# garrelt/C2-Ray3Dm1D_Helium

Measured on AMD Instinct MI355X. Metric: cell-updates/sec (grid_cells x sources x iters / wall) on 256^3 box; % HBM roofline, higher is better.
Workload: dtype f64

## Files before the change

### __graft_entry__.py

```python
from __future__ import annotations

import importlib.util
import subprocess
import sys
from pathlib import Path

ROOT = Path(__file__).resolve().parent
PKG_DIR = ROOT / "c2-ray3dm1d_helium_amd"
PKG_NAME = "c2ray_helium_amd"
PARAMS_VARIANT = {"subboxsize": 4, "max_subbox": 9, "convergence_fraction": "1.0e-3"}


def load_package():
    if PKG_NAME in sys.modules:
        return sys.modules[PKG_NAME]
    spec = importlib.util.spec_from_file_location(PKG_NAME, PKG_DIR / "__init__.py",
                                                  submodule_search_locations=[str(PKG_DIR)])
    mod = importlib.util.module_from_spec(spec)
    sys.modules[PKG_NAME] = mod
    spec.loader.exec_module(mod)
    return mod


def build() -> None:
    pkg = load_package()
    lib = pkg.build(force=False)
    assert lib.exists(), lib
    subprocess.run(["make", "-C", str(ROOT / "oracle"), "liboracle.so", "liboracle_params.so"], check=True)
    alt = PKG_DIR / "libc2ray_hip_params.so"
    deps = pkg._build.SOURCES + pkg._build.HEADERS
    if not alt.exists() or alt.stat().st_mtime < max(p.stat().st_mtime for p in deps):
        pkg._build.build(params=PARAMS_VARIANT, out=alt)
    subprocess.run(["g++", "-O2", "-ffp-contract=off", "-mfma", "-fPIC", "-shared", "-std=c++17", "-o",
                    str(ROOT / "tests" / "_host_harness.so"), str(ROOT / "tests" / "host_harness.cpp")], check=True)
    from c2ray_helium_amd import _build
    for name, flags in (("gpu_func_probe", ["-O3"]), ("fake_rccl", ["-O2", "-pthread"]), ("fake_rccl_corrupt", ["-O2", "-pthread"])):
        src, so = ROOT / "tests" / f"{name}.hip", ROOT / "tests" / f"_{name}.so"
        deps = [src] + (list((PKG_DIR / "csrc").glob("*.hpp")) if name == "gpu_func_probe" else [])
        if name == "fake_rccl_corrupt":
            deps.append(ROOT / "tests" / "fake_rccl.hip")
        if not so.exists() or so.stat().st_mtime < max(p.stat().st_mtime for p in deps):
            subprocess.run([_build.hipcc(), "--offload-arch=gfx950", *flags, "-ffp-contract=off", "-fPIC", "-shared", "-std=c++17", "-o",
                            str(so), str(src)], check=True)
    for variant in (["16"], ["16", "pl"], ["16", "lls"], ["16", "cubep3m"], ["16", "params"], ["64", "omp"], ["256", "omp", "timer"]):
        subprocess.run([str(ROOT / "oracle" / "ref_build.sh"), *variant], check=True)
    import ctypes
    so = ctypes.CDLL(str(lib))
    for name in pkg._lib.SYMBOLS:
        getattr(so, name)


def smoke() -> None:
    import numpy as np
    pkg = load_package()
    sys.path.insert(0, str(ROOT / "oracle"))
    import oracle as orc

    z = np.load(ROOT / "tests" / "golden" / "tap_N16_heat_3src.npz")
    g = lambda k: z["c1_in_" + k]
    tables = pkg.RadiationTables.load()
    mesh = tuple(int(m) for m in g("mesh"))
    mat = pkg.Material(ndens=g("ndens"), xh=g("xh").copy(), xhe=g("xhe").copy(),
                       temperature_grid=g("temperature").copy(), isothermal=False,
                       temper_val=float(g("temper_val")[0]), clumping=float(g("clumping")[0]), reccoef=g("reccoef"))
    grid = pkg.GridProps(mesh, tuple(g("dr")), float(g("vol")[0]))
    src = pkg.SourceProps(g("srcpos").reshape(-1, 3), g("NormFlux"), float(g("S_star")[0]))
    cosmo = pkg.Cosmology(float(g("zred")[0]), float(g("H0")[0]), float(g("Omega0")[0]))
    ev = pkg.Evolve(mesh, tables, device=0)
    e = ev.engine
    e.set_step(mat, grid, cosmo)
    e.set_sources(src)
    e.upload_state(mat)
    e.begin_step()
    e.set_rates_to_zero()
    e.pass_sources(1, 1)
    conv = e.global_pass(float(g("dt")[0]))
    got = {**e.download_rates(), **e.download_iter_state()}

    with np.load(pkg.evolve.DEFAULT_TABLES) as t:
        T = orc.Tables({k: t[k] for k in t.files})
    st = orc.Step(mesh, g("dr"), g("vol")[0], g("zred")[0], g("H0")[0], g("Omega0")[0], 0, g("temper_val")[0],
                  g("clumping")[0], g("srcpos"), g("NormFlux"), g("S_star")[0], g("ndens"), g("reccoef"))
    s = orc.State(st, g("xh"), g("xhe"), g("temperature"))
    orc.begin_step(s)
    orc.pass_all_sources(T, st, s)
    conv_ref = orc.global_pass(T, st, s, float(g("dt")[0]))
    worst = 0.0
    for k, ref in [("phih_grid", s.phih), ("phihe_grid", s.phihe), ("phiheat", s.phiheat), ("xh_av", s.xh_av),
                   ("xhe_av", s.xhe_av), ("xh_intermed", s.xh_intermed)]:
        rel = np.abs(got[k] - ref) / np.maximum(np.abs(ref), 1e-300)
        worst = max(worst, float(rel.max()))
    print(f"smoke: 16^3 x 3 sources, heating: conv_flag gpu={conv} oracle={conv_ref}, worst rel diff {worst:.3e}")
    assert conv == conv_ref, (conv, conv_ref)
    assert worst == 0.0, worst


if __name__ == "__main__":
    build()
    print("build ok")
```

### c2-ray3dm1d_helium_amd/csrc/c2ray_hip.hip

```cpp
#include <hip/hip_runtime.h>

#include <algorithm>
#include <atomic>
#include <chrono>
#include <cmath>
#include <cstdarg>
#include <cstdio>
#include <cstdlib>
#include <cstring>
#include <string>
#include <thread>
#include <type_traits>
#include <unordered_map>
#include <vector>

#include "../../include/c2ray_hip.h"
#include "c2ray_device.hpp"
#include "c2ray_shell.hpp"

using namespace c2r;

namespace {

constexpr int BATCH_MAX = 4096;
// ... 341 lines not shown
  const StepScalars &sc = A.sc;
  int di, dj, dk;
  ReachShell RS{};
  if constexpr (OPEN) RS = reach_shell(S.rl, S.rr, G.s);
  const int face = OPEN ? reach_decode(RS, t, di, dj, dk) : shell_decode_fast(G, t, di, dj, dk);
  Box cut_;
  if constexpr (OPEN) cut_ = source_box(A.box, S);
  const Box &box = OPEN ? cut_ : A.box;
  const bool inside = di >= box.lo[0] && di <= box.hi[0] && dj >= box.lo[1] && dj <= box.hi[1] && dk >= box.lo[2] &&
                      dk <= box.hi[2];
  if (!inside) return;
  const size_t cz = S.cz;
  const size_t p = (OPEN ? (size_t)RS.off : (size_t)G.off) + (size_t)t;
  global_double *cs = (global_double *)S.cols;
  const int i = mesh0<OPEN>(S.i0 - 1 + di, g.n1), j = mesh0<OPEN>(S.j0 - 1 + dj, g.n2), k = mesh0<OPEN>(S.k0 - 1 + dk, g.n3);
  double u_HI, u_HeI, u_HeII;
  sweep_cell_state(A, i, j, k, face == 2, u_HI, u_HeI, u_HeII);
  ShellCorners c4;
  if constexpr (OPEN) reach_short_characteristic(G, reach_shell(S.rl, S.rr, G.sp), S.rl, S.rr, face, S.i0, S.j0, S.k0, di, dj, dk, c4);
  else shell_short_characteristic(G, face, S.i0, S.j0, S.k0, di, dj, dk, c4);
  double cin_HI = interp_column_fast(c4.s, cs[col_out((size_t)c4.p[0], 0, cz)], cs[col_out((size_t)c4.p[1], 0, cz)],
                                     cs[col_out((size_t)c4.p[2], 0, cz)], cs[col_out((size_t)c4.p[3], 0, cz)], sigma_HI_at_ion_freq);
  const double cin_HeI = interp_column_fast(c4.s, cs[col_out((size_t)c4.p[0], 1, cz)], cs[col_out((size_t)c4.p[1], 1, cz)],
                                            cs[col_out((size_t)c4.p[2], 1, cz)], cs[col_out((size_t)c4.p[3], 1, cz)], sigma_HeI_at_ion_freq);
  const double cin_HeII = interp_column_fast(c4.s, cs[col_out((size_t)c4.p[0], 2, cz)], cs[col_out((size_t)c4.p[1], 2, cz)],
                                             cs[col_out((size_t)c4.p[2], 2, cz)], cs[col_out((size_t)c4.p[3], 2, cz)], sigma_HeII_at_ion_freq);
  const double path = c4.path * sc.dr1;
  if (sc.use_lls) {
    const double coldensh_LLS =
        A.lls_grid ? (double)A.lls_grid[(size_t)i + (size_t)g.n1 * ((size_t)j + (size_t)g.n2 * (size_t)k)] : sc.coldensh_lls;
    cin_HI = cin_HI + coldensh_LLS * path / sc.dr1;
  }
  const double cout_HI = cin_HI + u_HI * path * (1.0 - abu_he);
  const double cout_HeI = cin_HeI + u_HeI * path * abu_he;
  const double cout_HeII = cin_HeII + u_HeII * path * abu_he;
  store_columns(cs, p, cz, cin_HI, cin_HeI, cin_HeII, cout_HI, cout_HeI, cout_HeII);
}

__device__ __forceinline__ int sweep_block_cell(int cnt) {
  const int nblk_shell = (cnt + BLOCK - 1) / BLOCK;
  int vb = (int)blockIdx.x;
  if ((gridDim.x & 7u) == 0) {
    const int chunk = (int)gridDim.x >> 3;
    vb = ((int)blockIdx.x & 7) * chunk + ((int)blockIdx.x >> 3);
  }
  if (vb >= nblk_shell) return -1;
  const int t = vb * BLOCK + (int)threadIdx.x;
  return t < cnt ? t : -1;
}

__device__ __forceinline__ int sweep_block_cell_open(int cnt) {
  const int nblk_shell = (cnt + BLOCK - 1) / BLOCK;
  int vb = (int)blockIdx.x;
  if (nblk_shell >= 64) {
    const int chunk = (nblk_shell + 7) >> 3;
    if (vb >= 8 * chunk) return -1;
    vb = (vb & 7) * chunk + (vb >> 3);
  }
  if (vb >= nblk_shell) return -1;
  const int t = vb * BLOCK + (int)threadIdx.x;
  return t < cnt ? t : -1;
}

template <bool OPEN>
__device__ __forceinline__ int sweep_shell_cells(const SrcDev &S, int shell) {
  if constexpr (OPEN) return (int)(reach_cells(S.rl, S.rr, shell) - reach_cells(S.rl, S.rr, shell - 1));
  else return (int)shell_count(shell);
}

template <bool OPEN>
__global__ void __launch_bounds__(BLOCK, C2R_SWEEP_WAVES)
k_sweep_shell(SweepArgs A, const SrcDev *__restrict__ src, const int *__restrict__ active, int shell) {
  const SrcDev &S = src[active[blockIdx.y]];
  const int t = OPEN ? sweep_block_cell_open(sweep_shell_cells<OPEN>(S, shell)) : sweep_block_cell((int)shell_count(shell));
  if (t >= 0) sweep_cell<OPEN>(A, S, shell, t);
}

template <bool OPEN>
__global__ void __launch_bounds__(BLOCK, C2R_SWEEP_WAVES)
k_sweep_shell_fast(SweepArgs A, const SrcDev *__restrict__ src, const int *__restrict__ active, ShellGeom G) {
  const SrcDev &S = src[active[blockIdx.y]];
  const int t = OPEN ? sweep_block_cell_open(sweep_shell_cells<OPEN>(S, G.s)) : sweep_block_cell(24 * G.s * G.s + 2);
  if (t >= 0) sweep_cell_fast<OPEN>(A, S, G, t);
}

__global__ void __launch_bounds__(BLOCK)
k_loss_finish(const double *__restrict__ loss_partial, int pitch, int count, double *__restrict__ loss_acc) {
  __shared__ double sh[BLOCK / 64];
  const double *p = loss_partial + (size_t)blockIdx.x * pitch;
  double a = 0.0;
  for (int i = threadIdx.x; i < count; i += BLOCK) a += p[i];
  const double tot = block_sum(a, sh);
  if (threadIdx.x == 0) loss_acc[blockIdx.x] = tot;
}

struct ProbeRound {
  int s_lo, s_hi;
  Box box;
  int list_off;
  int nact;
  int nblk;
  int partial_off;
  int acc_off;
};
template <bool OPEN>
__global__ void __launch_bounds__(BLOCK)
k_loss_probe_rounds(Grid g, const SrcDev *__restrict__ src, const int *__restrict__ lists, const ProbeRound *__restrict__ rounds,
                    int multi, StepScalars sc, const BandData *__restrict__ bd, SedSet ss, const int *__restrict__ block_base,
                    double *__restrict__ loss_partial, int sample) {
  __shared__ double sh[BLOCK / 64];
  const ProbeRound &R = rounds[blockIdx.z];
  if ((int)blockIdx.x >= R.nblk || (int)blockIdx.y >= R.nact) return;
  const SrcDev &S = src[lists[R.list_off + blockIdx.y]];
  Box cut_;
  if constexpr (OPEN) cut_ = source_box(R.box, S);
  const Box &box = OPEN ? cut_ : R.box;
  const int s_lo = R.s_lo, s_hi = R.s_hi;
  const int B = block_base[s_hi + 1] - 1 - (int)blockIdx.x * sample;
  int lo = s_lo, hi = s_hi;
  while (lo < hi) {
    const int mid = (lo + hi + 1) >> 1;
    if (block_base[mid] <= B) lo = mid; else hi = mid - 1;
  }
  const int shell = lo;
  ReachShell RS{};
  if constexpr (OPEN) RS = reach_shell(S.rl, S.rr, shell);
  const long long cnt = OPEN ? (long long)RS.cnt : shell_count(shell);
  const int slot = threadIdx.x & 31;
  const long long t = (long long)(B - block_base[shell]) * BLOCK + (threadIdx.x >> 5) * 32;
  double loss = 0.0;
  if (t < cnt) {
    int di, dj, dk;
    if constexpr (OPEN) reach_decode(RS, (int)t, di, dj, dk);
    else shell_decode(shell, (int)t, di, dj, dk);
    const bool inside = di >= box.lo[0] && di <= box.hi[0] && dj >= box.lo[1] && dj <= box.hi[1] && dk >= box.lo[2] &&
                        dk <= box.hi[2];
    const bool boundary = on_counted_face<OPEN>(box, S, di, dj, dk, 1);
    if (inside && boundary) {
      const size_t cz = S.cz;
      const size_t p = (OPEN ? (size_t)RS.off : (size_t)shell_offset(shell)) + (size_t)t;
      const global_double *cs = (const global_double *)S.cols;
      const double cin_HI = cs[col_in(p, 0, cz)], cin_HeI = cs[col_in(p, 1, cz)], cin_HeII = cs[col_in(p, 2, cz)];
      const double cout_HI = cs[col_out(p, 0, cz)], cout_HeI = cs[col_out(p, 1, cz)], cout_HeII = cs[col_out(p, 2, cz)];
      if (cin_HI < max_coldensh) {
        double vol_ph;
        if (shell == 0) {
          vol_ph = sc.dr1 * sc.dr2 * sc.dr3;
        } else {
          const double path = sc_path(di, dj, dk) * sc.dr1;
          const double xs = sc.dr1 * (double)di, ys = sc.dr2 * (double)dj, zs = sc.dr3 * (double)dk;
          vol_ph = 4.0 * pi * (xs * xs + ys * ys + zs * zs) * path;
        }
        const double nf[NSED] = {S.nflux, S.nflux_sed[0], S.nflux_sed[1]};
        double po = 0.0;
        for (int sd = 0; sd < (multi ? NSED : 1); sd++) {
          if (!(nf[sd] > 0.0)) continue;
          for (int b = ss.lo[sd] + slot; b < ss.hi[sd]; b += 32)
            po += photo_out_band(*bd, sd, ss.photo_thick[sd], ss.photo_thin[sd], b, cin_HI, cout_HI, cin_HeI, cout_HeI, cin_HeII,
                                 cout_HeII, nf[sd]);
        }
        loss = po * sc.vol / vol_ph;
      }
    }
  }
  const double bs = block_sum(loss, sh);
  if (threadIdx.x == 0) loss_partial[(size_t)R.partial_off + (size_t)blockIdx.y * R.nblk + blockIdx.x] = bs;
// ... 2112 lines not shown
  }
  HIPCHK(c, hipMemcpyAsync(c->d_src[set], hs, sizeof(SrcDev) * B.nb, hipMemcpyHostToDevice, c->stream));
  return 0;
}

static int settle_rounds(const PassCtx &P, Batch &B) {
  c2r_ctx *c = P.c;
  if (B.settled == B.recs.size()) return 0;
  if (launch_probes(P, B)) return 1;
  HIPCHK(c, hipEventSynchronize(c->ev_probe));
  int *hl = c->h_list[B.set];
  for (; B.settled < B.recs.size(); B.settled++) {
    const RoundRec &R = B.recs[B.settled];
    const double *probe = c->h_probe + R.acc_off;
    const int *lst = hl + R.off;
    std::vector<int> undecided;
    for (int a = 0; a < R.nact; a++) {
      SrcRun &r = B.run[lst[a]];
      if (!r.active) continue;
      r.loss = probe[a];
      if (!(r.loss > 2.0 * (C2R_F(1e-10) * r.total_flux))) undecided.push_back(lst[a]);
    }
    if (!undecided.empty()) {
      int *ul = hl + B.list_used;
      std::copy(undecided.begin(), undecided.end(), ul);
      HIPCHK(c, hipMemcpyAsync(c->d_list[B.set] + B.list_used, ul, sizeof(int) * undecided.size(), hipMemcpyHostToDevice, c->stream));
      if (boundary_loss(c, B.set, B.list_used, (int)undecided.size(), R.s_lo, R.s_hi, R.box, P.sc, P.ss, P.multi, true)) return 1;
      B.list_used += undecided.size();
      for (size_t j = 0; j < undecided.size(); j++) B.run[undecided[j]].loss = c->h_loss[j];
    }
    for (int a = 0; a < R.nact; a++) {
      SrcRun &r = B.run[lst[a]];
      if (!r.active) continue;
      if (!(r.loss > C2R_F(1e-10) * r.total_flux)) {
        r.active = false;
        r.nbox = R.round;
      }
    }
  }
  return 0;
}

static bool all_reached(const c2r_ctx *c, const Batch &B, int round) {
  for (const SrcRun &r : B.run)
    if (r.active && c->prev_nbox[(size_t)r.ns - 1] < round) return false;
  return true;
}

static int move_block(const PassCtx &P, Batch &B, int b, int ncap, double *ncols) {
  c2r_ctx *c = P.c;
  SrcRun &r = B.run[b];
  if (B.launched > B.settled) HIPCHK(c, hipStreamWaitEvent(c->stream, c->ev_probe, 0));
  SrcDev &S = c->h_src[B.set][b];
  const size_t ncz = source_block_entries(c, r.ns, ncap);
  const size_t have = r.smax_prev >= 0 ? source_block_entries(c, r.ns, r.smax_prev) : 0;
  for (int half = 0; half < 2 && have > 0; half++)
    HIPCHK(c, hipMemcpyAsync(ncols + 3 * half * ncz, S.cols + 3 * half * S.cz, sizeof(double) * 3 * have,
                             hipMemcpyDeviceToDevice, c->stream));
  if (S.cz > 0) c->vacated[B.set].push_back(c2r_ctx::Segment{S.cols, 6 * S.cz});
  S.cols = ncols;
  S.cz = ncz;
  r.cap = ncap;
  c->arena_stats[3]++;
  HIPCHK(c, hipMemcpyAsync(c->d_src[B.set] + b, &S, sizeof(SrcDev), hipMemcpyHostToDevice, c->stream));
  return 0;
}

static int start_over(const PassCtx &P, Batch &B, int round) {
  c2r_ctx *c = P.c;
  HIPCHK(c, hipStreamSynchronize(c->stream));
  HIPCHK(c, hipStreamSynchronize(c->stream_probe));
  const int limit_rounds = (c->g.smax + SUBBOXSIZE - 1) / SUBBOXSIZE;
  for (const SrcRun &r : B.run) {
    int &pn = c->prev_nbox[(size_t)r.ns - 1];
    pn = std::max(pn, r.active ? limit_rounds : r.nbox);
  }
  if (B.nb == 1) return fail(c, "column scratch: one source of this mesh does not fit in device memory");
  if (P.arena_log) fprintf(stderr, "c2ray_hip: column scratch, set %d: no room to grow in round %d, batch of %d starts over\n", B.set, round, B.nb);
  if (B.restarts++ > 0) B.nb = (B.nb + 1) / 2;
  c->arena_stats[4]++;
  return START_OVER;
}

static int launch_shells(PassCtx &P, Batch &B, const Box &box, int s_lo, int s_hi, size_t act_off, int nact) {
  c2r_ctx *c = P.c;
  SweepArgs SA;
  SA.g = c->g; SA.box = box; SA.sc = P.sc;
  SA.ndens = c->d_ndens; SA.xh_av = c->d_xh_av; SA.xhe_av = c->d_xhe_av;
  SA.lls_grid = c->lls_on_grid ? c->d_lls : nullptr;
  const int *act = c->h_list[B.set] + act_off;
  if (c->timing && !B.sweep_started) {
    HIPCHK(c, hipEventRecord(B.ev[0], c->stream));
    B.sweep_started = true;
  }
  for (int s = s_lo; s <= s_hi; s++) {
    if ((s >= TRANSPOSED_FROM_SHELL || B.nb > 16) && !P.transposed_seen) {
      HIPCHK(c, hipStreamWaitEvent(c->stream, c->ev_transposed, 0));
      P.transposed_seen = true;
    }
    SA.packed = SA.packedT = nullptr;
    if (P.transposed_seen || P.packed_early) SA.packed = c->d_stateT;
    if (P.transposed_seen) SA.packedT = c->d_stateT + 3 * c->g.ncell;
    int nblk = c->block_base[s + 1] - c->block_base[s];
    if (!c->periodic) {
      long long most = 0;
      for (int a = 0; a < nact; a++) {
        const Reach &R = B.run[act[a]].reach;
        most = std::max(most, reach_cells(R.l, R.r, s) - reach_cells(R.l, R.r, s - 1));
      }
      nblk = (int)((most + BLOCK - 1) / BLOCK);
      if (nblk == 0) continue;
    }
    const int nlaunch = nblk >= 64 ? ((nblk + 7) & ~7) : nblk;
    for (int a = 0; a < nact; a++)
      if (s <= B.run[act[a]].smax) B.run[act[a]].sweep_threads += (long long)nlaunch * BLOCK;
    const bool fast = s >= 2 && (s <= SHELL_FAST_MAX || !c->periodic) && !P.generic_sweep;
    if (fast && c->periodic)
      hipLaunchKernelGGL(k_sweep_shell_fast<false>, dim3(nlaunch, nact), dim3(BLOCK), 0, c->stream, SA, c->d_src[B.set],
                         c->d_list[B.set] + act_off, c->shell_geom[(size_t)s]);
    else if (fast)
      hipLaunchKernelGGL(k_sweep_shell_fast<true>, dim3(nlaunch, nact), dim3(BLOCK), 0, c->stream, SA, c->d_src[B.set],
                         c->d_list[B.set] + act_off, c->shell_geom[(size_t)s]);
    else if (c->periodic)
      hipLaunchKernelGGL(k_sweep_shell<false>, dim3(nlaunch, nact), dim3(BLOCK), 0, c->stream, SA, c->d_src[B.set], c->d_list[B.set] + act_off, s);
    else
      hipLaunchKernelGGL(k_sweep_shell<true>, dim3(nlaunch, nact), dim3(BLOCK), 0, c->stream, SA, c->d_src[B.set], c->d_list[B.set] + act_off, s);
    c->tm.sweep_launches++;
  }
  HIPCHK(c, hipGetLastError());
  return 0;
}

static int sweep_batch(PassCtx &P, Batch &B) {
  c2r_ctx *c = P.c;
  const Reach &reach = P.reach;
  B.list_used = 0;
  B.recs.clear();
  B.settled = B.launched = 0;
  B.sweep_started = false;
  const size_t acc_need = (size_t)B.nb * (size_t)(c->g.smax / SUBBOXSIZE + 3);
  if (c->probe_acc_cap < acc_need) {
    HIPCHK(c, hipStreamSynchronize(c->stream_probe));
    if (ensure_pair<double>(c, &c->d_probe_acc, &c->h_probe, &c->probe_acc_cap, acc_need)) return 1;
  }
  int *hl = c->h_list[B.set];
  size_t cur_off = 0;
  int cur_nact = 0;
  size_t acc_used = 0;
  for (int round = 1;; round++) {
    const Box box = round_box(reach, round);
    int s_hi = 0;
    const bool ahead = round > 1 && cur_nact > 0 && all_reached(c, B, round);
    if (!ahead && settle_rounds(P, B)) return 1;
    int nact = 0;
    int *act = hl + B.list_used;
    int s_lo = 1 << 30;
    for (int b = 0; b < B.nb; b++) {
      SrcRun &r = B.run[b];
      if (!r.active) continue;
      if (!can_grow(c, r.reach, round_box(r.reach, r.nbox)) || !(ahead || r.loss > C2R_F(1e-10) * r.total_flux)) {
        r.active = false;
        continue;
      }
      r.nbox = round;
      act[nact++] = b;
      s_lo = std::min(s_lo, r.smax_prev + 1);
      s_hi = std::max(s_hi, box_smax(round_box(r.reach, round)));
    }
    if (nact == 0) return settle_rounds(P, B);
    if (s_hi > c->g.smax) return fail(c, "internal: shell %d beyond smax %d", s_hi, c->g.smax);
    for (int a = 0; a < nact; a++) {
      const int cap = B.run[act[a]].cap;
      const int need = std::min(s_hi, B.run[act[a]].smax);
      if (cap >= need) continue;
      const int ncap = std::min(B.run[act[a]].smax, std::max(need, 2 * cap));
      double *ncols = arena_alloc(c, B.set, source_block_doubles(c, B.run[act[a]].ns, ncap));
      if (!ncols) return start_over(P, B, round);
      if (move_block(P, B, act[a], ncap, ncols)) return 1;
    }
    size_t act_off = B.list_used;
    if (cur_nact == nact && round > 1 && std::equal(act, act + nact, hl + cur_off)) {
      act_off = cur_off;
    } else {
      HIPCHK(c, hipMemcpyAsync(c->d_list[B.set] + B.list_used, act, sizeof(int) * nact, hipMemcpyHostToDevice, c->stream));
      B.list_used += (size_t)nact;
    }
    cur_off = act_off;
    cur_nact = nact;
    if (launch_shells(P, B, box, s_lo, s_hi, act_off, nact)) return 1;
    bool any_can_grow = false, any_can_grow_twice = false;
    for (int a = 0; a < nact; a++) {
      SrcRun &r = B.run[hl[act_off + a]];
      r.smax_prev = std::min(s_hi, r.smax);
      any_can_grow = any_can_grow || can_grow(c, r.reach, round_box(r.reach, round));
      any_can_grow_twice = any_can_grow_twice || can_grow(c, r.reach, round_box(r.reach, round + 1));
    }
    if (!any_can_grow) {
      if (settle_rounds(P, B)) return 1;
      for (int a = 0; a < nact; a++) {
        SrcRun &r = B.run[hl[act_off + a]];
        if (!r.active) continue;
        r.final_loss_due = true;
        r.active = false;
      }
      return 0;
    }
    RoundRec R;
    R.round = round; R.nact = nact; R.s_lo = s_lo; R.s_hi = s_hi; R.off = act_off; R.acc_off = acc_used; R.box = box;
    acc_used += (size_t)nact;
    B.recs.push_back(R);
// ... 1122 lines not shown
```

### c2-ray3dm1d_helium_amd/csrc/c2ray_shell.hpp

```cpp
#pragma once

#include <stdint.h>

#include "c2ray_device.hpp"

namespace c2r {

C2R_HD long long shell_count(int s) { return s == 0 ? 1 : 24LL * s * s + 2; }

C2R_HD long long shell_offset(int s) { return s == 0 ? 0 : (long long)(2 * s - 1) * (2 * s - 1) * (2 * s - 1); }

C2R_HD void shell_decode(int s, int t, int &di, int &dj, int &dk) {
  if (s == 0) { di = dj = dk = 0; return; }
  const int w = 2 * s + 1, v = 2 * s - 1;
  const int A = w * w, B = v * w, C = v * v;
  if (t < 2 * A) {
    dk = t < A ? s : -s;
    if (t >= A) t -= A;
    dj = t / w - s;
    di = t % w - s;
  } else if (t < 2 * A + 2 * B) {
    t -= 2 * A;
    dj = t < B ? s : -s;
    if (t >= B) t -= B;
// ... 69 lines not shown
  const int s = G.s;
  const int face = t < 2 * G.A ? 0 : (t < 2 * G.A + 2 * G.B ? 1 : 2);
  const int first = face == 0 ? 0 : (face == 1 ? 2 * G.A : 2 * G.A + 2 * G.B);
  const int size = face == 0 ? G.A : (face == 1 ? G.B : G.C);
  const int width = face == 2 ? G.v : G.w;
  const uint32_t magic = face == 2 ? G.mv : G.mw;
  const int shift = face == 2 ? G.kv : G.kw;
  const int tf = t - first;
  const bool neg = tf >= size;
  const uint32_t u = (uint32_t)(neg ? tf - size : tf);
  const uint32_t r = mulhi_u32(u, magic) >> shift;
  const int col = (int)(u - r * (uint32_t)width);
  const int a = col - (face == 2 ? s - 1 : s);
  const int b = (int)r - (face == 0 ? s : s - 1);
  const int c = neg ? -s : s;
  di = face == 2 ? c : a;
  dj = face == 0 ? b : (face == 1 ? c : a);
  dk = face == 0 ? c : b;
  return face;
}

C2R_HD int position_in_previous_shell(const ShellGeom &G, int i, int j, int k) {
  const int sp = G.sp;
  const int ja = j < 0 ? -j : j, ka = k < 0 ? -k : k;
  const int tk = (k > 0 ? 0 : G.Ap) + (j + sp) * G.wp + (i + sp);
  const int tj = 2 * G.Ap + (j > 0 ? 0 : G.Bp) + (k + sp - 1) * G.wp + (i + sp);
  const int ti = 2 * G.Ap + 2 * G.Bp + (i > 0 ? 0 : G.Cp) + (k + sp - 1) * G.vp + (j + sp - 1);
  return ka == sp ? tk : (ja == sp ? tj : ti);
}

struct ShellCorners {
  uint32_t p[4];
  double s[4];
  double path;
};
C2R_HD void shell_short_characteristic(const ShellGeom &G, int face, int i0, int j0, int k0, int di, int dj, int dk,
                                       ShellCorners &sc) {
  const int sp = G.sp;
  const int da = face == 2 ? dj : di, db = face == 0 ? dj : dk;
  const int a0 = face == 2 ? j0 : i0, b0 = face == 0 ? j0 : k0;
  const int sga = da >= 0 ? 1 : -1, sgb = db >= 0 ? 1 : -1;
  const int am = da - sga, bm = db - sgb;
  const double fa = (double)da, fb = (double)db;
  const double ac = G.alam * fa + (double)a0, bc = G.alam * fb + (double)b0;
  const double ea = 2.0 * fabs(ac - ((double)(a0 + am) + 0.5 * sga));
  const double eb = 2.0 * fabs(bc - ((double)(b0 + bm) + 0.5 * sgb));
  sc.s[0] = (1. - ea) * (1. - eb);
  sc.s[1] = (1. - eb) * ea;
  sc.s[2] = (1. - ea) * eb;
  sc.s[3] = ea * eb;
  const double num = fa * fa + fb * fb;
  const double q0 = num * G.rn2;
  const double quo = __builtin_fma(__builtin_fma(-G.n2, q0, num), G.rn2, q0);
  sc.path = sqrt(quo + 1.0);
  const int ca = da > sp ? sp : (da < -sp ? -sp : da), cb = db > sp ? sp : (db < -sp ? -sp : db);
  const uint32_t offp = (uint32_t)G.offp;
  if (face == 0) {
    const int km = dk > 0 ? sp : -sp;
    const int base = (km > 0 ? 0 : G.Ap) + sp;
    const int ra = base + (bm + sp) * G.wp, rb = base + (cb + sp) * G.wp;
    sc.p[0] = offp + (uint32_t)(ra + am);
    sc.p[1] = offp + (uint32_t)(ra + ca);
    sc.p[2] = offp + (uint32_t)(rb + am);
    sc.p[3] = offp + (uint32_t)(rb + ca);
  } else if (face == 1) {
    const int jm = dj > 0 ? sp : -sp;
    const int rk_base = (jm + sp) * G.wp + sp, rj_base = 2 * G.Ap + (jm > 0 ? 0 : G.Bp) + sp + (sp - 1) * G.wp;
    const int bma = bm < 0 ? -bm : bm, cba = cb < 0 ? -cb : cb;
    const int ra = bma == sp ? (bm > 0 ? 0 : G.Ap) + rk_base : rj_base + bm * G.wp;
    const int rb = cba == sp ? (cb > 0 ? 0 : G.Ap) + rk_base : rj_base + cb * G.wp;
    sc.p[0] = offp + (uint32_t)(ra + am);
    sc.p[1] = offp + (uint32_t)(ra + ca);
    sc.p[2] = offp + (uint32_t)(rb + am);
    sc.p[3] = offp + (uint32_t)(rb + ca);
  } else {
    const int im = di > 0 ? sp : -sp;
    sc.p[0] = offp + (uint32_t)position_in_previous_shell(G, im, am, bm);
    sc.p[1] = offp + (uint32_t)position_in_previous_shell(G, im, ca, bm);
    sc.p[2] = offp + (uint32_t)position_in_previous_shell(G, im, am, cb);
    sc.p[3] = offp + (uint32_t)position_in_previous_shell(G, im, ca, cb);
  }
}

C2R_HD int reach_lo(int l, int s) { return l > -s ? l : -s; }
C2R_HD int reach_hi(int r, int s) { return r < s ? r : s; }
C2R_HD long long reach_cells(const int *l, const int *r, int s) {
  if (s < 0) return 0;
  long long e = 1;
  for (int d = 0; d < 3; d++) e *= (long long)(reach_hi(r[d], s) - reach_lo(l[d], s) + 1);
  return e;
}

struct ReachShell {
  int s;
  int lox, loy;
  int loyp, lozp;
  int ex, eyp;
  int b1, b2, b3, b4, b5;
  int cnt;
  uint32_t off;
};
C2R_HD ReachShell reach_shell(const int *l, const int *r, int s) {
  ReachShell G;
  G.s = s;
  G.lox = reach_lo(l[0], s);
  G.loy = reach_lo(l[1], s);
  G.ex = reach_hi(r[0], s) - G.lox + 1;
  const int ey = reach_hi(r[1], s) - G.loy + 1;
  if (s == 0) {
    G.loyp = G.lozp = 0;
    G.eyp = 1;
    G.b1 = G.b2 = G.b3 = G.b4 = G.b5 = G.cnt = 1;
    G.off = 0;
    return G;
  }
  G.loyp = reach_lo(l[1], s - 1);
  G.lozp = reach_lo(l[2], s - 1);
  G.eyp = reach_hi(r[1], s - 1) - G.loyp + 1;
  const int exp_ = reach_hi(r[0], s - 1) - reach_lo(l[0], s - 1) + 1;
  const int ezp = reach_hi(r[2], s - 1) - G.lozp + 1;
  const int A = G.ex * ey, B = G.ex * ezp, C = G.eyp * ezp;
  G.b1 = s <= r[2] ? A : 0;
  G.b2 = G.b1 + (s <= -l[2] ? A : 0);
  G.b3 = G.b2 + (s <= r[1] ? B : 0);
  G.b4 = G.b3 + (s <= -l[1] ? B : 0);
  G.b5 = G.b4 + (s <= r[0] ? C : 0);
  G.cnt = G.b5 + (s <= -l[0] ? C : 0);
  G.off = (uint32_t)(exp_ * G.eyp * ezp);
  return G;
}

C2R_HD int reach_decode(const ReachShell &G, int t, int &di, int &dj, int &dk) {
  const int s = G.s;
  const int face = t < G.b2 ? 0 : (t < G.b4 ? 1 : 2);
  const int first = face == 0 ? 0 : (face == 1 ? G.b2 : G.b4);
  const int mid = face == 0 ? G.b1 : (face == 1 ? G.b3 : G.b5);
  const int width = face == 2 ? G.eyp : G.ex;
  const bool neg = t >= mid;
  const uint32_t u = (uint32_t)(t - (neg ? mid : first));
  const uint32_t row = u / (uint32_t)width;
  const int col = (int)(u - row * (uint32_t)width);
  const int a = col + (face == 2 ? G.loyp : G.lox);
  const int b = (int)row + (face == 0 ? G.loy : G.lozp);
  const int c = neg ? -s : s;
  di = face == 2 ? c : a;
  dj = face == 0 ? b : (face == 1 ? c : a);
  dk = face == 0 ? c : b;
  return face;
}

C2R_HD int reach_position_in_shell(const ReachShell &G, int i, int j, int k) {
  const int s = G.s;
  const int ja = j < 0 ? -j : j, ka = k < 0 ? -k : k;
  const int tk = (k > 0 ? 0 : G.b1) + (j - G.loy) * G.ex + (i - G.lox);
  const int tj = (j > 0 ? G.b2 : G.b3) + (k - G.lozp) * G.ex + (i - G.lox);
  const int ti = (i > 0 ? G.b4 : G.b5) + (k - G.lozp) * G.eyp + (j - G.loyp);
  return s == 0 ? 0 : (ka == s ? tk : (ja == s ? tj : ti));
}

C2R_HD size_t reach_position(const int *l, const int *r, int di, int dj, int dk) {
  const int ia = di < 0 ? -di : di, ja = dj < 0 ? -dj : dj, ka = dk < 0 ? -dk : dk;
  const int s = ia > ja ? (ia > ka ? ia : ka) : (ja > ka ? ja : ka);
  const ReachShell G = reach_shell(l, r, s);
  return (size_t)G.off + (size_t)reach_position_in_shell(G, di, dj, dk);
}

// ... 63 lines not shown
```

Measured before the change: 5.909 billion.

## Fuse groups of consecutive shells into one blocked sweep kernel with LDS hand-off

Adds a kernel that processes K (2 or 4) consecutive shells per launch for periodic fast sweeps. Each block owns a tile of the outermost shell, recomputes its upstream halo on inner shells, and passes column densities between shells through shared memory instead of reloading them from global memory. This cuts the number of kernel launches and the global traffic for the upstream columns. The cost is redundant halo recomputation and extra shared-memory use, which may lower occupancy.

```diff
diff --git a/__graft_entry__.py b/__graft_entry__.py
--- a/__graft_entry__.py
+++ b/__graft_entry__.py
@@ -31,8 +31,9 @@
     deps = pkg._build.SOURCES + pkg._build.HEADERS
     if not alt.exists() or alt.stat().st_mtime < max(p.stat().st_mtime for p in deps):
         pkg._build.build(params=PARAMS_VARIANT, out=alt)
-    subprocess.run(["g++", "-O2", "-ffp-contract=off", "-mfma", "-fPIC", "-shared", "-std=c++17", "-o",
-                    str(ROOT / "tests" / "_host_harness.so"), str(ROOT / "tests" / "host_harness.cpp")], check=True)
+    for name in ("host_harness", "sweep_blocked_harness"):
+        subprocess.run(["g++", "-O2", "-ffp-contract=off", "-mfma", "-fPIC", "-shared", "-std=c++17", "-o",
+                        str(ROOT / "tests" / f"_{name}.so"), str(ROOT / "tests" / f"{name}.cpp")], check=True)
     from c2ray_helium_amd import _build
     for name, flags in (("gpu_func_probe", ["-O3"]), ("fake_rccl", ["-O2", "-pthread"]), ("fake_rccl_corrupt", ["-O2", "-pthread"])):
         src, so = ROOT / "tests" / f"{name}.hip", ROOT / "tests" / f"_{name}.so"
diff --git a/c2-ray3dm1d_helium_amd/csrc/c2ray_hip.hip b/c2-ray3dm1d_helium_amd/csrc/c2ray_hip.hip
--- a/c2-ray3dm1d_helium_amd/csrc/c2ray_hip.hip
+++ b/c2-ray3dm1d_helium_amd/csrc/c2ray_hip.hip
@@ -447,6 +447,111 @@
   const SrcDev &S = src[active[blockIdx.y]];
   const int t = OPEN ? sweep_block_cell_open(sweep_shell_cells<OPEN>(S, G.s)) : sweep_block_cell(24 * G.s * G.s + 2);
   if (t >= 0) sweep_cell_fast<OPEN>(A, S, G, t);
+}
+
+template <int K>
+struct ShellGroup { ShellGeom G[K]; };
+
+__device__ __forceinline__ int sweep_block_tile(int ntiles) {
+  int vb = (int)blockIdx.x;
+  if ((gridDim.x & 7u) == 0) {
+    const int chunk = (int)gridDim.x >> 3;
+    vb = ((int)blockIdx.x & 7) * chunk + ((int)blockIdx.x >> 3);
+  }
+  return vb < ntiles ? vb : -1;
+}
+
+template <bool FIRST>
+__device__ __forceinline__ void sweep_cell_blocked(const SweepArgs &A, const SrcDev &S, const ShellGeom &G, int f, int a, int b, int c,
+                                                   bool owned, const double *in, int in_pitch, const PatchRect &P, double &o_HI,
+                                                   double &o_HeI, double &o_HeII) {
+  const Grid &g = A.g;
+  const StepScalars &sc = A.sc;
+  const Box &box = A.box;
+  int di, dj, dk;
+  plane_cell(f, a, b, c, di, dj, dk);
+  o_HI = o_HeI = o_HeII = 0.0;
+  const bool inside = di >= box.lo[0] && di <= box.hi[0] && dj >= box.lo[1] && dj <= box.hi[1] && dk >= box.lo[2] &&
+                      dk <= box.hi[2];
+  if (!inside) return;
+  const int face = shell_face(G, dj, dk);
+  const size_t cz = S.cz;
+  global_double *cs = (global_double *)S.cols;
+  const int i = wrap0(S.i0 - 1 + di, g.n1), j = wrap0(S.j0 - 1 + dj, g.n2), k = wrap0(S.k0 - 1 + dk, g.n3);
+  double u_HI, u_HeI, u_HeII;
+  sweep_cell_state(A, i, j, k, f == 2, u_HI, u_HeI, u_HeII);
+  ShellCorners c4;
+  shell_short_characteristic(G, face, S.i0, S.j0, S.k0, di, dj, dk, c4);
+  double n[3][4];
+  if constexpr (FIRST) {
+#pragma unroll
+    for (int x = 0; x < 3; x++)
+#pragma unroll
+      for (int q = 0; q < 4; q++) n[x][q] = cs[col_out((size_t)c4.p[q], x, cz)];
+  } else {
+    int slot[4];
+    shell_corner_slots(G, face, f, P, di, dj, dk, slot);
+#pragma unroll
+    for (int x = 0; x < 3; x++)
+#pragma unroll
+      for (int q = 0; q < 4; q++) n[x][q] = in[x * in_pitch + slot[q]];
+  }
+  double cin_HI = interp_column_fast(c4.s, n[0][0], n[0][1], n[0][2], n[0][3], sigma_HI_at_ion_freq);
+  const double cin_HeI = interp_column_fast(c4.s, n[1][0], n[1][1], n[1][2], n[1][3], sigma_HeI_at_ion_freq);
+  const double cin_HeII = interp_column_fast(c4.s, n[2][0], n[2][1], n[2][2], n[2][3], sigma_HeII_at_ion_freq);
+  const double path = c4.path * sc.dr1;
+  if (sc.use_lls) {
+    const double coldensh_LLS =
+        A.lls_grid ? (double)A.lls_grid[(size_t)i + (size_t)g.n1 * ((size_t)j + (size_t)g.n2 * (size_t)k)] : sc.coldensh_lls;
+    cin_HI = cin_HI + coldensh_LLS * path / sc.dr1;
+  }
+  o_HI = cin_HI + u_HI * path * (1.0 - abu_he);
+  o_HeI = cin_HeI + u_HeI * path * abu_he;
+  o_HeII = cin_HeII + u_HeII * path * abu_he;
+  if (owned && face == f)
+    store_columns(cs, (size_t)G.off + (size_t)position_in_shell(G, di, dj, dk), cz, cin_HI, cin_HeI, cin_HeII, o_HI, o_HeI, o_HeII);
+}
+
+template <int K>
+__global__ void __launch_bounds__(BLOCK, 6)
+k_sweep_shells_blocked(SweepArgs A, const SrcDev *__restrict__ src, const int *__restrict__ active, ShellGroup<K> GG) {
+  constexpr int TA = SWEEP_TILE_A, TB = sweep_tile_b(K);
+  constexpr int N0 = sweep_patch_cells(K, K - 1), N1 = K > 2 ? sweep_patch_cells(K, K - 2) : 1;
+  static_assert(N0 <= 2 * BLOCK && 3 * (N0 + N1) * sizeof(double) <= 16384, "two handed-over shells in 16 KB");
+  __shared__ double hand0[3 * N0], hand1[3 * N1];
+  const SrcDev &S = src[active[blockIdx.y]];
+  const int s_last = GG.G[K - 1].s;
+  const int tile = sweep_block_tile(sweep_tile_count(s_last, TA, TB));
+  if (tile < 0) return;
+  int f, sgn;
+  PatchRect T;
+  sweep_tile(s_last, TA, TB, tile, f, sgn, T);
+#pragma unroll 1
+  for (int m = 0; m < K; m++) {
+    const ShellGeom &G = GG.G[m];
+    PatchRect Q = T;
+    for (int s = s_last; s > G.s; s--) Q = upstream_rect(Q, s - 1);
+    const PatchRect P = upstream_rect(Q, G.sp);
+    const int na = Q.ahi - Q.alo + 1, cells = na * (Q.bhi - Q.blo + 1);
+    const uint32_t magic = patch_magic(na);
+    double *out = (m & 1) ? hand1 : hand0;
+    const double *in = (m & 1) ? hand0 : hand1;
+    const int out_pitch = (m & 1) ? N1 : N0, in_pitch = (m & 1) ? N0 : N1;
+    for (int idx = (int)threadIdx.x; idx < cells; idx += BLOCK) {
+      const int row = patch_row(idx, magic);
+      const int a = Q.alo + (idx - row * na), b = Q.blo + row;
+      const bool owned = a >= T.alo && a <= T.ahi && b >= T.blo && b <= T.bhi;
+      double o_HI, o_HeI, o_HeII;
+      if (m == 0) sweep_cell_blocked<true>(A, S, G, f, a, b, sgn * G.s, owned, in, in_pitch, P, o_HI, o_HeI, o_HeII);
+      else sweep_cell_blocked<false>(A, S, G, f, a, b, sgn * G.s, owned, in, in_pitch, P, o_HI, o_HeI, o_HeII);
+      if (m < K - 1) {
+        out[idx] = o_HI;
+        out[out_pitch + idx] = o_HeI;
+        out[2 * out_pitch + idx] = o_HeII;
+      }
+    }
+    if (m < K - 1) __syncthreads();
+  }
 }
 
 __global__ void __launch_bounds__(BLOCK)
@@ -2725,6 +2830,20 @@
   return START_OVER;
 }
 
+struct SweepBlocking { int from, K; };
+static const SweepBlocking SWEEP_BLOCKING[] = {{2, 4}, {64, 1}};
+static int sweep_blocking_row(int s) {
+  int r = 0;
+  for (int i = 0; i < (int)(sizeof SWEEP_BLOCKING / sizeof SWEEP_BLOCKING[0]); i++)
+    if (s >= SWEEP_BLOCKING[i].from) r = i;
+  return r;
+}
+static int sweep_blocking(int s) { return s < SWEEP_BLOCKING[0].from ? 1 : SWEEP_BLOCKING[sweep_blocking_row(s)].K; }
+static int sweep_blocking_end(int s) {
+  const int r = sweep_blocking_row(s), n = (int)(sizeof SWEEP_BLOCKING / sizeof SWEEP_BLOCKING[0]);
+  return r + 1 < n ? SWEEP_BLOCKING[r + 1].from - 1 : SHELL_FAST_MAX;
+}
+
 static int launch_shells(PassCtx &P, Batch &B, const Box &box, int s_lo, int s_hi, size_t act_off, int nact) {
   c2r_ctx *c = P.c;
   SweepArgs SA;
@@ -2736,8 +2855,15 @@
     HIPCHK(c, hipEventRecord(B.ev[0], c->stream));
     B.sweep_started = true;
   }
-  for (int s = s_lo; s <= s_hi; s++) {
-    if ((s >= TRANSPOSED_FROM_SHELL || B.nb > 16) && !P.transposed_seen) {
+  for (int s = s_lo; s <= s_hi;) {
+    int K = 1;
+    if (c->periodic && !P.generic_sweep && s >= 2) {
+      const int want = sweep_blocking(s);
+      const int room = std::min(std::min(s_hi, SHELL_FAST_MAX), sweep_blocking_end(s)) - s + 1;
+      K = want >= 4 && room >= 4 ? 4 : (want >= 2 && room >= 2 ? 2 : 1);
+    }
+    const int s_end = s + K - 1;
+    if ((s_end >= TRANSPOSED_FROM_SHELL || B.nb > 16) && !P.transposed_seen) {
       HIPCHK(c, hipStreamWaitEvent(c->stream, c->ev_transposed, 0));
       P.transposed_seen = true;
     }
@@ -2745,6 +2871,7 @@
     if (P.transposed_seen || P.packed_early) SA.packed = c->d_stateT;
     if (P.transposed_seen) SA.packedT = c->d_stateT + 3 * c->g.ncell;
     int nblk = c->block_base[s + 1] - c->block_base[s];
+    if (K > 1) nblk = sweep_tile_count(s_end, SWEEP_TILE_A, sweep_tile_b(K));
     if (!c->periodic) {
       long long most = 0;
       for (int a = 0; a < nact; a++) {
@@ -2752,13 +2879,23 @@
         most = std::max(most, reach_cells(R.l, R.r, s) - reach_cells(R.l, R.r, s - 1));
       }
       nblk = (int)((most + BLOCK - 1) / BLOCK);
-      if (nblk == 0) continue;
+      if (nblk == 0) { s++; continue; }
     }
     const int nlaunch = nblk >= 64 ? ((nblk + 7) & ~7) : nblk;
     for (int a = 0; a < nact; a++)
-      if (s <= B.run[act[a]].smax) B.run[act[a]].sweep_threads += (long long)nlaunch * BLOCK;
+      if (s <= B.run[act[a]].smax) B.run[act[a]].sweep_threads += (long long)nlaunch * BLOCK * K;
     const bool fast = s >= 2 && (s <= SHELL_FAST_MAX || !c->periodic) && !P.generic_sweep;
-    if (fast && c->periodic)
+    if (K == 4) {
+      ShellGroup<4> GG;
+      for (int m = 0; m < 4; m++) GG.G[m] = c->shell_geom[(size_t)(s + m)];
+      hipLaunchKernelGGL(k_sweep_shells_blocked<4>, dim3(nlaunch, nact), dim3(BLOCK), 0, c->stream, SA, c->d_src[B.set],
+                         c->d_list[B.set] + act_off, GG);
+    } else if (K == 2) {
+      ShellGroup<2> GG;
+      for (int m = 0; m < 2; m++) GG.G[m] = c->shell_geom[(size_t)(s + m)];
+      hipLaunchKernelGGL(k_sweep_shells_blocked<2>, dim3(nlaunch, nact), dim3(BLOCK), 0, c->stream, SA, c->d_src[B.set],
+                         c->d_list[B.set] + act_off, GG);
+    } else if (fast && c->periodic)
       hipLaunchKernelGGL(k_sweep_shell_fast<false>, dim3(nlaunch, nact), dim3(BLOCK), 0, c->stream, SA, c->d_src[B.set],
                          c->d_list[B.set] + act_off, c->shell_geom[(size_t)s]);
     else if (fast)
@@ -2769,6 +2906,7 @@
     else
       hipLaunchKernelGGL(k_sweep_shell<true>, dim3(nlaunch, nact), dim3(BLOCK), 0, c->stream, SA, c->d_src[B.set], c->d_list[B.set] + act_off, s);
     c->tm.sweep_launches++;
+    s = s_end + 1;
   }
   HIPCHK(c, hipGetLastError());
   return 0;
diff --git a/c2-ray3dm1d_helium_amd/csrc/c2ray_shell.hpp b/c2-ray3dm1d_helium_amd/csrc/c2ray_shell.hpp
--- a/c2-ray3dm1d_helium_amd/csrc/c2ray_shell.hpp
+++ b/c2-ray3dm1d_helium_amd/csrc/c2ray_shell.hpp
@@ -175,6 +175,89 @@
   }
 }
 
+constexpr int SWEEP_TILE_A = 16;
+C2R_HD constexpr int sweep_tile_b(int K) { return K <= 2 ? 16 : 14; }
+C2R_HD constexpr int sweep_patch_cells(int K, int back) { return (SWEEP_TILE_A + back) * (sweep_tile_b(K) + back); }
+
+struct PatchRect { int alo, ahi, blo, bhi; };
+C2R_HD int clamp_int(int x, int lo, int hi) { return x < lo ? lo : (x > hi ? hi : x); }
+
+C2R_HD int upstream_lo(int lo, int sp) { return lo > 0 ? lo - 1 : (lo < -sp ? -sp : lo); }
+C2R_HD int upstream_hi(int hi, int sp) { return hi < 0 ? hi + 1 : (hi > sp ? sp : hi); }
+C2R_HD PatchRect upstream_rect(const PatchRect &R, int sp) {
+  return PatchRect{upstream_lo(R.alo, sp), upstream_hi(R.ahi, sp), upstream_lo(R.blo, sp), upstream_hi(R.bhi, sp)};
+}
+
+C2R_HD void sweep_tile_counts(int s, int ta, int tb, int &nk, int &nj, int &ni) {
+  const int w = 2 * s + 1, v = 2 * s - 1;
+  const int aw = (w + ta - 1) / ta, av = (v + ta - 1) / ta, bw = (w + tb - 1) / tb, bv = (v + tb - 1) / tb;
+  nk = aw * bw; nj = aw * bv; ni = av * bv;
+}
+C2R_HD int sweep_tile_count(int s, int ta, int tb) {
+  int nk, nj, ni;
+  sweep_tile_counts(s, ta, tb, nk, nj, ni);
+  return 2 * (nk + nj + ni);
+}
+
+C2R_HD void sweep_tile(int s, int ta, int tb, int tile, int &f, int &sgn, PatchRect &R) {
+  int nk, nj, ni;
+  sweep_tile_counts(s, ta, tb, nk, nj, ni);
+  f = tile < 2 * nk ? 0 : (tile < 2 * nk + 2 * nj ? 1 : 2);
+  const int first = f == 0 ? 0 : (f == 1 ? 2 * nk : 2 * nk + 2 * nj), size = f == 0 ? nk : (f == 1 ? nj : ni);
+  int u = tile - first;
+  sgn = u < size ? 1 : -1;
+  if (u >= size) u -= size;
+  const int ea = f == 2 ? 2 * s - 1 : 2 * s + 1, eb = f == 0 ? 2 * s + 1 : 2 * s - 1;
+  const int na = (ea + ta - 1) / ta;
+  const int row = u / na, col = u - row * na;
+  const int a0 = -(ea / 2), b0 = -(eb / 2);
+  R.alo = a0 + col * ta;
+  R.blo = b0 + row * tb;
+  R.ahi = R.alo + ta - 1 < -a0 ? R.alo + ta - 1 : -a0;
+  R.bhi = R.blo + tb - 1 < -b0 ? R.blo + tb - 1 : -b0;
+}
+
+C2R_HD uint32_t patch_magic(int n) { return (65536u + (uint32_t)n - 1u) / (uint32_t)n; }
+C2R_HD int patch_row(int idx, uint32_t magic) { return (int)(((uint32_t)idx * magic) >> 16); }
+
+C2R_HD void plane_cell(int f, int a, int b, int c, int &di, int &dj, int &dk) {
+  di = f == 2 ? c : a;
+  dj = f == 0 ? b : (f == 1 ? c : a);
+  dk = f == 0 ? c : b;
+}
+
+C2R_HD int shell_face(const ShellGeom &G, int dj, int dk) {
+  const int ja = dj < 0 ? -dj : dj, ka = dk < 0 ? -dk : dk;
+  return ka == G.s ? 0 : (ja == G.s ? 1 : 2);
+}
+
+C2R_HD int position_in_shell(const ShellGeom &G, int i, int j, int k) {
+  const int s = G.s;
+  const int ja = j < 0 ? -j : j, ka = k < 0 ? -k : k;
+  const int tk = (k > 0 ? 0 : G.A) + (j + s) * G.w + (i + s);
+  const int tj = 2 * G.A + (j > 0 ? 0 : G.B) + (k + s - 1) * G.w + (i + s);
+  const int ti = 2 * G.A + 2 * G.B + (i > 0 ? 0 : G.C) + (k + s - 1) * G.v + (j + s - 1);
+  return ka == s ? tk : (ja == s ? tj : ti);
+}
+
+C2R_HD void shell_corner_slots(const ShellGeom &G, int face, int f, const PatchRect &P, int di, int dj, int dk, int (&slot)[4]) {
+  const int sp = G.sp;
+  const int da = face == 2 ? dj : di, db = face == 0 ? dj : dk, dc = face == 0 ? dk : (face == 1 ? dj : di);
+  const int am = da - (da >= 0 ? 1 : -1), bm = db - (db >= 0 ? 1 : -1);
+  const int ca = da > sp ? sp : (da < -sp ? -sp : da), cb = db > sp ? sp : (db < -sp ? -sp : db);
+  const int cm = dc > 0 ? sp : -sp;
+  const int na = P.ahi - P.alo + 1;
+#if defined(__clang__)
+#pragma unroll
+#endif
+  for (int c = 0; c < 4; c++) {
+    int ci, cj, ck;
+    plane_cell(face, (c & 1) ? ca : am, (c & 2) ? cb : bm, cm, ci, cj, ck);
+    const int a = clamp_int(f == 2 ? cj : ci, P.alo, P.ahi), b = clamp_int(f == 0 ? cj : ck, P.blo, P.bhi);
+    slot[c] = (b - P.blo) * na + (a - P.alo);
+  }
+}
+
 C2R_HD int reach_lo(int l, int s) { return l > -s ? l : -s; }
 C2R_HD int reach_hi(int r, int s) { return r < s ? r : s; }
 C2R_HD long long reach_cells(const int *l, const int *r, int s) {
```

After: 5.932 billion, median of 6. About the same (+0.4%).
